# ajzhai/PEANUT

Hardware: AMD Instinct MI355X
Metric: maps/sec for 480x480x(4+N_cat) prediction fwd, batch 32 (higher is better)
Workload: dtype f32; 1 GPU; 480x480, 14-channel (4+10) partial maps -> 6-class prediction forward (PSPNet R50-V1c-D8), batch 32 per GPU, seeded random-init weights; survey_config=2, global_batch=32, parallelism=dp1 (map shards, no data-path collective)

## Files before the change

### peanut_amd/csrc/common.h

```cpp
#pragma once
#include <hip/hip_runtime.h>
#include <stdint.h>
#include <string>

#include "persistent_plan.h"

namespace peanut {

void set_error(const std::string& msg);
int fail(int code, const std::string& msg);
void note_kernel(const char* family);
const char* noted_kernel();

#define PEANUT_HIP_CHECK(expr)                                                            \
  do {                                                                                    \
    hipError_t _e = (expr);                                                               \
    if (_e != hipSuccess)                                                                 \
      return ::peanut::fail(-3, std::string(#expr) + ": " + hipGetErrorString(_e));       \
  } while (0)

struct ConvDesc {
  int cin;
  int cout;
  int kh, kw, stride, pad, dil;
// ... 94 lines not shown
  int pack_bn;
  int G;
  PersistentPlan plan;
  int code;
  const char* error;
};
struct ConvKParams;
ConvRoute conv_route(const ConvDesc& d, const ConvArgs& a, ConvKParams* params = nullptr);
ConvRoute conv_route_patch_nchw();
const char* conv_kernel_family(const ConvRoute& r);
int device_cus();
bool conv_pw_enabled();
bool conv_pw_uses_256(int cout, long long M, int mt_per_group, int bn_tile, int cin);
int conv_pw_256_min_k();
bool conv_pw_uses_256w(int cout, long long M, int mt_per_group, int bn_tile, int cin, int flush_ktiles);
bool conv_pw_narrow_tiles(int cin, int cout, long long M, int bn_tile, int mt_per_group);
bool conv_pw_uses_256p(int cout, long long M, int mt_per_group, int bn_tile, int cin, int flush_ktiles, long long in_pixels = 0);
bool gemm_skinny_takes(const ConvKParams& p, int bn_tile, size_t ws_floats);
bool conv_pw_uses_256wp(int cout, long long M, int stride, int mt_per_group, int bn_tile, int c1, int c2, int flush_ktiles);
bool conv_pw_uses_ares(int cin, int cout, long long M, int stride, bool two_source, int flush_ktiles, int bn_tile);

bool conv_patch_eligible(const ConvDesc& d, const ConvArgs& a);
bool conv_patch_nchw_eligible(const ConvDesc& d, int B, int Ho, int Wo, int creal);
int launch_conv_patch_nchw(const ConvDesc& d, const float* x_nchw, int creal, float* y, int B, int H, int W, int Ho, int Wo, hipStream_t stream);

void wino_geometry(int B, int H, int W, int dil, int* th, int* tw, long long* n_tiles, long long* m_pad, int gran = 128, int m = 4);
void wino_transform_weights(const float* w_oihw, int cout, int cin, float* out, int m = 4);
int launch_wino_input(const float* x, float* V, int B, int H, int W, int C, int dil, hipStream_t s, int gran = 128, int m = 4, long long m_pad_total = 0,
                      const DeferredSplit* df = nullptr);
bool wino_input_accepts_deferred(int B, int H, int W, int C, int dil, int gran, int m);
long long wino_deferred_count();
int launch_wino_output(const float* Mb, const float* scale, const float* shift, const float* res, float* y,
                       int B, int H, int W, int C, int dil, int relu, hipStream_t s, int gran = 128, int m = 4, long long m_pad_total = 0);

bool gemm_rs_uses_256(int cout, long long M, int mt_per_group, int bn_tile, int cin);
bool gemm_rs_uses_64(int cout, long long M, int bn_tile, int cin);
size_t sx_packed_bytes(int cin_pad, int cout, int bn_tile, int planes);
void pack_weights_sx(const float* w, int cout, int cin_real, int cin_pad, int bn_tile, int planes, float wscale, void* out);
float sx_pack_scale(const float* w, size_t n, int planes);
size_t sx_conv_packed_bytes(int cin_pad, int cout, int kh, int kw, int bn_tile, int planes);
void pack_weights_sx_conv(const float* w_oihw, int cout, int cin_real, int cin_pad, int kh, int kw, int bn_tile, int planes,
                          float wscale, void* out);

int launch_nchw_to_nhwc_pad(const float* x, float* y, int B, int C, int H, int W, int Cpad, hipStream_t s);
int launch_maxpool3x3s2(const float* x, float* y, int B, int H, int W, int C, int Ho, int Wo, hipStream_t s);
int launch_ppm_pool(const float* x, float* out, int B, int H, int W, int C, const int* scales, int nscales,
                    hipStream_t s, int scale_rows = 0);
size_t ppm_pool_scratch_floats(int B, int H, int C, const int* scales, int nscales);
int launch_ppm_pool2(const float* x, float* scratch, float* out, int B, int H, int W, int C, const int* scales,
                     int nscales, hipStream_t s, int scale_rows = 0);
int launch_ppm_upsample_concat(const float* table, float* out, int B, int H, int W, int Cp, const int* scales,
                               int nscales, int align_corners, hipStream_t s);
int launch_ppm_conv_term(const float* Q, float* R, int B, int H, int W, int C, const int* scales, int nscales,
                         int align_corners, hipStream_t s, int scale_rows = 0);
int launch_upsample_logits(const float* lo, float* out, int B, int h, int w, int K, int H, int W,
                           int align_corners, int sigmoid, hipStream_t s);

}
```

### peanut_amd/csrc/options.h

```cpp
#pragma once
#include <stdlib.h>
#include <string.h>

#include <string>

namespace peanut {

enum OptionId {
  OPT_PW_GLDS, OPT_PW256_MINK, OPT_PW256_MINTILES, OPT_PW256_PHASE, OPT_PW256_SKIP_PAD, OPT_PW256W_MINK, OPT_PW256W_MINTILES, OPT_PW256P_MINK, OPT_PW256P_MINTILES, OPT_PW256P_FLUSH, OPT_PW256P_ORDER, OPT_PW256P_STREAMK, OPT_PW256WP_MINK, OPT_PW256WP_MINTILES, OPT_PW256WP_NPRE, OPT_PW256WP_STAGGER, OPT_PW_ARES, OPT_PW_SKINNY,
  OPT_PW_ARES_MINUNITS, OPT_PATCH_MINTILES, OPT_STEM_NCHW, OPT_BN64_MAXK, OPT_PW_BN64_MAXK, OPT_PW64_MAXTILES, OPT_FP32_BK, OPT_NCHUNK, OPT_RES_PREFETCH, OPT_SPLIT_MODEL,
  OPT_RS_CONV, OPT_RS_BN64_MAXK, OPT_RS256_MINK, OPT_RS256_MINTILES, OPT_RS64_MAXK, OPT_RS64_MAXTILES,
  OPT_WINO_M, OPT_WINO_HEAD_M, OPT_WINO6_MAXDIL, OPT_WINO5_MINDIL, OPT_WINO_FLUSH_CH, OPT_WINO_MIN_CIN, OPT_WINO_NARROW_MINPIX, OPT_WINO_SMALL_MAXWG, OPT_DEFER_SPLITK,
  OPT_PPM_OVERLAP, OPT_PPM_GROUPED, OPT_PPM_TERM_ROWS, OPT_PPM_GROUP_ROWS, OPT_RCNN_WINO_M, OPT_RCNN_STEM_S2D, OPT_RCNN_RPN_FUSED, OPT_RCNN_FPN_OVERLAP, OPT_RCNN_RANK_SORT, OPT_RCNN_TOPK_SLICE, OPT_RCNN_NMS_LEVELS, OPT_FMM_LOCAL32, OPT_FMM_MAX_PASSES, OPT_FMM_BLOCKED, OPT_FMM_INNER,
  OPT_DEBUG_POISON_ALLOC,
  OPT_COUNT
};

struct OptionInfo {
  const char* key;
  long long def;
  bool upload_time;
  const char* help;
};

inline const OptionInfo* option_table() {
  static const OptionInfo t[OPT_COUNT] = {
      {"pw_glds", 1, false, "fp32 1x1 convs / grouped GEMMs on the LDS-DMA kernels of conv_pw.hip (0: conv_igemm)"},
      {"pw256_mink", 1024, false, "fewest input channels for the 256 x 128 three-stage kernel"},
      {"pw256_mintiles", 256, false, "fewest 256 x 128 tiles for that kernel"},
      {"pw256_phase", 1, false, "the two waves of a SIMD request their LDS-DMA pieces half an iteration apart"},
      {"pw256_skip_pad", 1, false, "256 x 128 kernel, grouped GEMMs: waves whose rows are all group padding issue no MFMAs (0: compute the zero rows)"},
      {"pw256w_mink", 768, false, "fewest input channels for the 256 x 256 two-stage kernel (0: off)"},
      {"pw256w_mintiles", 1536, false, "fewest 256 x 256 tiles for that kernel"},
      {"pw256p_mink", 512, false, "fewest input channels for the persistent 256 x 128 kernel (conv_pw256p.hip; 0: off)"},
      {"pw256p_mintiles", 512, false, "fewest 256 x 128 tiles for that kernel"},
      {"pw256p_flush", 512, false, "most input channels of a Winograd position GEMM (two-level accumulation) that runs on the persistent kernel (0: none)"},
      {"pw256p_order", 1, false, "persistent 256 x 128 kernel: 1 = the workgroups of an XCD walk its run of tiles side by side (neighbours share operand panels in L2), 0 = one contiguous run per workgroup"},
      {"pw256p_streamk", 1, false, "persistent 256 x 128 kernel: the tail tiles' k-tiles as one stream in equal runs per workgroup (0: every tail tile cut into the same number of parts)"},
      {"pw256wp_mink", 512, false, "fewest input channels for the persistent 256 x 256 kernel (conv_pw256wp.hip; 0: off)"},
      {"pw256wp_mintiles", 768, false, "fewest 256 x 256 tiles for that kernel"},
      {"pw256wp_npre", 0, false, "persistent 256 x 256 kernel: accumulator blocks per in-place epilogue group (2 or 4; 0 = two with a residual, four without)"},
      {"pw256wp_stagger", 0, false, "persistent 256 x 256 kernel: spread of the workgroups' start times in sleeps of ~3.4 us (their tile boundaries -- 512 KiB of epilogue traffic per CU -- then fall at different times)"},
      {"pw_ares", 1, false, "K = 128 / 256 pointwise layers on the persistent A-resident kernel (conv_pw_ares.hip)"},
      {"pw_skinny", 1, false, "grouped pointwise launches with at most 64 data rows per group (the PSP pyramid's per-scale convs and Q tables at batch 1) on the skinny weight-streaming kernel (gemm_skinny.hip: 6 KiB of LDS, fits next to any other kernel; 0: the MFMA kernels on 128-row padded tiles)"},
      {"pw_ares_minunits", 512, false, "fewest (m-tile, n-tile) units for that kernel"},
      {"patch_mintiles", 1024, false, "3x3 convs of 16 / 32 input channels on the persistent LDS-patch kernel (conv_patch.hip) from this many 8 x 16 output tiles (0: off)"},
      {"stem_nchw", 1, false, "prediction forward: the first stem conv reads the NCHW input itself (conv_patch.hip, NCHW variant) instead of a layout pass + NHWC conv (fp32 mode, when the patch kernel takes the layer)"},
      {"bn64_maxk", 256, true, "128 x 64 tiles for layers with at most this many input channels"},
      {"pw_bn64_maxk", 128, true, "pointwise layers / Winograd position GEMMs: weights PACKED 64 wide up to this many input channels (wider layers: 128-wide packing, 64-wide tiles chosen per shape)"},
      {"pw64_maxtiles", 512, false, "a 128-wide-packed pointwise layer with at most bn64_maxk input channels runs 128 x 64 tiles while its 128 x 128 tiling has fewer tiles than this (two per CU)"},
      {"fp32_bk", 0, true, "16: force 16-channel k-tiles in conv_igemm (experiment)"},
      {"nchunk", 8, false, "n-tiles per chunk of the tile order (0: n fastest over all n-tiles)"},
      {"res_prefetch", 1, false, "request the first residual rows before the last k-tile's MFMAs"},
      {"split_model", 1, false, "tail split-K plan counts CUs (1) or resident slots (0)"},
      {"rs_conv", 1, true, "emulated modes: non-pointwise convs on conv_rs.hip (0: fp32 MFMA kernel)"},
      {"rs_bn64_maxk", 128, true, "emulated modes: 128 x 64 tiles up to this many input channels"},
      {"rs256_mink", 512, false, "emulated modes: fewest input channels for the 256 x 256 kernel"},
      {"rs256_mintiles", 256, false, "emulated modes: fewest 256 x 256 tiles for it"},
      {"rs64_maxk", 512, false, "emulated modes: 64 x 64 tiles up to this many input channels"},
      {"rs64_maxtiles", 128, false, "emulated modes: ... and below this many 128-row tiles"},
      {"wino_m", 0, true, "4 / 5 / 6: force one Winograd form on every eligible layer (0: policy)"},
      {"wino_head_m", 0, true, "4 / 5 / 6: Winograd form of the PSP bottleneck (0: policy)"},
      {"wino6_maxdil", 4, true, "largest dilation that gets an F(6x6) form"},
      {"wino5_mindil", 4, true, "smallest dilation that also gets an F(5x5) form (0: none)"},
      {"wino_flush_ch", 64, true, "channels per partial sum of the position GEMMs' two-level accumulation (0: off)"},
      {"wino_min_cin", 0, true, "fewest input channels of a Winograd layer (0: the planner's policy)"},
      {"wino_narrow_minpix", 20000, false, "layers under 128 channels take their Winograd form from this many input pixels on (round 6: 100 000 -> 20 000 -- with the small-problem transforms one 720 x 720 map's layer1 conv2, 32 400 pixels, gains 5 us per layer as F(6x6); profiles/r9e)"},
      {"wino_small_maxwg", 1024, false, "Winograd transforms: launches with fewer workgroups than this of the one-thread-per-tile kernels take the small-problem variants (a workgroup per tile and 64-channel slice, a thread per line, through LDS; bit-identical; 0: never)"},
      {"defer_splitk", 1, false, "a Bottleneck conv1 whose every tile is split along k leaves its partial tiles unsummed and conv2's (small-problem) Winograd input transform sums them: one launch fewer per block at batch 1, bit-identical (0: every conv runs its own reduce); read when a (B, H, W) plan is built"},
      {"ppm_overlap", -1, false, "pyramid branch of the PSP head on a side stream: 0 / 1, -1 = by size"},
      {"ppm_grouped", -1, false, "per-scale PSP GEMMs as one grouped launch: 0 / 1, -1 = by size"},
      {"ppm_term_rows", 1, false, "folded pyramid term: one wave per output row, no barrier in the row loop (0: the workgroup-wide two-phase kernel)"},
      {"ppm_group_rows", 0, false, "pyramid pooling, row pass: rows added up per workgroup (1..5; 0 = by size: as many as still leave ~768 workgroups)"},
      {"rcnn_wino_m", 0, true, "detector front end: 4 / 5 / 6 pins one Winograd form (0: per shape)"},
      {"rcnn_stem_s2d", 1, true, "detector stem 7x7 stride 2 as a space-to-depth 4x4 conv"},
      {"rcnn_rpn_fused", 1, false, "detector: the RPN head on all five pyramid levels as one chain (five input transforms, ONE grouped Winograd GEMM, five output transforms, one objectness and one anchor-delta GEMM over all levels' rows: 12 launches instead of 25); read when a (B, H, W) plan is built"},
      {"rcnn_fpn_overlap", 0, false, "detector: the FPN output convs of p5, p4, p3 on a side stream next to the lateral / top-down chain that ends in p2's (round 5 experiment, bit-identical; measured SLOWER at batch 1, 5.70 against 5.61 ms per frame, profiles/r8: off); read when a (B, H, W) plan is built"},
      {"rcnn_rank_sort", 1, false, "detector: the RPN candidates of an image are ordered by counting the larger keys (n / 64 workgroups) instead of one workgroup's bitonic sort (round 5; same order: the keys are distinct)"},
      {"rcnn_topk_slice", 20480, false, "detector: objectness logits per workgroup of the per-level top-k (a level is cut into up to 8 ranges whose k largest are merged by counting; 0: one workgroup per level, round 4)"},
      {"rcnn_nms_levels", 1, false, "detector: the proposal NMS level by level (five 16 x 16-word suppression blocks and five scans per image side by side, post-NMS top-k by counting) instead of one score-sorted list per image (round 5; same proposals)"},
      {"fmm_local32", 1, false, "goal solver: single-precision local solve inside a tile"},
      {"fmm_max_passes", 24, false, "goal solver: hard ceiling of the second-order ordering passes; they stop as soon as a pass changes nothing (6-10 passes on the agent's 960 x 960 map; peanut_goal_converged reports whether they reached their fixed point)"},
      {"fmm_blocked", 1, false, "goal solver: a wave relaxes its 8 x 8 block of the tile to convergence between workgroup barriers (round 5; 0: one Jacobi sweep of the whole tile per barrier pair)"},
      {"fmm_inner", 48, false, "goal solver: iterations a wave spends on its block before it publishes it (blocked rounds)"},
      {"debug_poison_alloc", 0, false, "test switch: every device allocation the library makes for itself (workspace arenas, conv / Winograd / split-K scratch, the detector's and the goal solver's buffers, the map projection's arrays, uploaded weights before their copy) is filled with 0xFF bytes straight after hipMalloc -- fp32 / fp64 read NaN, int reads -1, 64-bit keys all ones -- so a kernel that reads a slot nothing wrote shows up as a changed result (tests/test_workspace_gpu.py); 0: allocations stay as the allocator returns them, no extra call"},
  };
  return t;
}

struct Options {
  long long v[OPT_COUNT];
};

inline int option_index(const char* key) {
  if (!key) return -1;
  std::string k(key);
  for (auto& c : k) c = (char)((c >= 'A' && c <= 'Z') ? c - 'A' + 'a' : c);
  if (k.rfind("peanut_", 0) == 0) k = k.substr(7);
  const OptionInfo* t = option_table();
  for (int i = 0; i < OPT_COUNT; ++i)
    if (k == t[i].key) return i;
  return -1;
}

inline Options& default_options() {
  static Options d = [] {
// ... 34 lines not shown
```

### peanut_amd/csrc/pred_api.hip

```cpp
#include <math.h>
#include <string.h>

#include <map>
#include <memory>
#include <string>
#include <vector>

#include "net_common.h"

namespace peanut {

static thread_local std::string g_err;
void set_error(const std::string& msg) { g_err = msg; }
int fail(int code, const std::string& msg) {
  g_err = msg;
  return code;
}
static thread_local const char* g_kernel = "";
void note_kernel(const char* family) { g_kernel = family; }
const char* noted_kernel() { return g_kernel; }

namespace {

enum OpKind { OP_TO_NHWC, OP_CONV, OP_CONV_NCHW, OP_MAXPOOL, OP_PPM_POOL, OP_PPM_UP, OP_PPM_TERM, OP_UPSAMPLE, OP_WINO_IN, OP_WINO_GEMM, OP_WINO_OUT };

struct Op {
  OpKind kind;
  std::string name;
  std::string kernel;
  const ConvLayer* conv = nullptr;
  Act in, in2, res, out;
  bool has_in2 = false, has_res = false;
  double flops = 0;
  double bytes = 0;
  int wino_mt_per_group = 0;
  int wino_valid_rows = 0;
  int wino_gran = 128;
  int branch = 0;
  bool fork_before = false, join_before = false;
  int group_mt = 0;
  int ppm_scale_rows = 0;
  bool defer_ok = false;
};

struct Plan {
  int B = 0, H = 0, W = 0;
  Act splitk;
  Act splitk2;
  bool keep_all = false;
  size_t bytes = 0;
  std::vector<Op> ops;
  std::map<std::string, Act> named;
};

}
}

using namespace peanut;

struct peanut_conv {
  Options opts = default_options();
  ConvLayer L;
  DevBuf ws;
  DevBuf wino_v, wino_m;
};

struct peanut_pred {
  Options opts = default_options();
  DeferredSplit deferred{};
  peanut_pred_cfg cfg{};
  int cin_pad = 0;
  std::vector<std::unique_ptr<ConvLayer>> convs;
  ConvLayer* stem[3] = {nullptr, nullptr, nullptr};
  struct Block { ConvLayer *c1, *c2, *c3, *down, *c3d; };
  std::vector<std::vector<Block>> layers;
  std::vector<ConvLayer*> ppm;
  ConvLayer* bottleneck = nullptr;
  ConvLayer* bottleneck_x = nullptr;
  std::vector<ConvLayer*> ppm_q;
  std::unique_ptr<ConvLayer> ppm_grouped, ppmq_grouped;
  ConvLayer* conv_seg = nullptr;
  int feat_channels = 0;
  bool keep_all = false;
  std::map<std::string, std::unique_ptr<Plan>> plans;
  Plan* last_plan = nullptr;
  DevBuf ws;
  bool use_graph = false;
  GraphCache graphs;
  bool probe = false;
  Plan* probe_plan = nullptr;
  std::vector<std::vector<hipEvent_t>> probe_events;
  std::vector<hipEvent_t> event_pool;
  hipStream_t side = nullptr;
  hipEvent_t ev_fork = nullptr, ev_join = nullptr;
  ~peanut_pred() {
    for (auto& v : probe_events) for (auto e : v) (void)hipEventDestroy(e);
    for (auto e : event_pool) (void)hipEventDestroy(e);
    if (ev_fork) (void)hipEventDestroy(ev_fork);
    if (ev_join) (void)hipEventDestroy(ev_join);
    if (side) (void)hipStreamDestroy(side);
  }
};

namespace {

int bn_fold(peanut_pred* h, const TensorMap& tm, const std::string& bn, int cout, float* scale, float* shift) {
  return bn_fold_eps(tm, bn, cout, h->cfg.bn_eps, scale, shift);
}

int add_conv(peanut_pred* h, const TensorMap& tm, const std::string& conv, const std::string& bn, int cin,
             int cin_pad, int cout, int k, int stride, int pad, int dil, int relu, ConvLayer** out) {
  int rc = 0;
  const int64_t wshape[4] = {cout, cin, k, k};
  const peanut_tensor* w = tm.get(conv + ".weight", 4, wshape, &rc);
// ... 271 lines not shown
      Act scr; scr.B = 1; scr.H = 1; scr.W = 1; scr.C = 0; scr.bytes = sf * sizeof(float); scr.off = ar.alloc(scr.bytes);
      op.in2 = scr; op.has_in2 = true;
      pl->ops.push_back(op);
      rel_side(scr);
    } else {
      pl->ops.push_back(op);
    }
  }
  Act table = make_act(ar, 1, 1, prow, h->cfg.head_channels);
  auto push_grouped = [&](const ConvLayer* G, const Act& in, const Act& out) {
    push_conv(*pl, G, in, nullptr, nullptr, out);
    Op& op = pl->ops.back();
    op.group_mt = srows / 128;
    op.flops = 2.0 * (double)prow * G->d.cout * G->cin_real;
  };
  if (srows) {
    push_grouped(h->ppm_grouped.get(), pooled, table);
  } else {
    size_t row0 = 0;
    for (int i = 0; i < h->cfg.n_pool_scales; ++i) {
      const int k = h->cfg.pool_scales[i];
      Act in = pooled, out = table;
      in.off = pooled.off + row0 * (size_t)x.C * sizeof(float);
      in.H = 1; in.W = k * k; in.C = x.C; in.B = B;
      out.off = table.off + row0 * (size_t)h->cfg.head_channels * sizeof(float);
      out.H = 1; out.W = k * k; out.C = h->cfg.head_channels; out.B = B;
      push_conv(*pl, h->ppm[i], in, nullptr, nullptr, out);
      row0 += (size_t)B * k * k;
    }
  }
  pl->named["ppm_table"] = table;
  rel_side(pooled);
  Act bt;
  int term_scale_rows = 0;
  if (h->bottleneck_x) {
    const int hc = h->cfg.head_channels;
    Act q = make_act(ar, 1, 1, prow, 9 * hc);
    if (srows) {
      push_grouped(h->ppmq_grouped.get(), table, q);
      term_scale_rows = srows;
    } else {
      size_t row0 = 0;
      for (int i = 0; i < h->cfg.n_pool_scales; ++i) {
        const int k = h->cfg.pool_scales[i];
        Act in = table, out = q;
        in.off = table.off + row0 * (size_t)hc * sizeof(float);
        in.H = 1; in.W = k * k; in.C = hc; in.B = B;
        out.off = q.off + row0 * (size_t)(9 * hc) * sizeof(float);
        out.H = 1; out.W = k * k; out.C = 9 * hc; out.B = B;
        push_conv(*pl, h->ppm_q[i], in, nullptr, nullptr, out);
        row0 += (size_t)B * k * k;
      }
    }
    rel_side(table);
    Act r = make_act(ar, B, x.H, x.W, hc);
    {
      Op op; op.kind = OP_PPM_TERM; op.name = "ppm_conv_term"; op.kernel = "ppm_conv_term"; op.in = q; op.out = r; op.ppm_scale_rows = term_scale_rows;
      op.bytes = (double)q.bytes + (double)r.bytes;
      pl->ops.push_back(op);
    }
    rel_side(q);
    const size_t side_end = pl->ops.size();
    bt = make_act(ar, B, x.H, x.W, h->bottleneck_x->d.cout);
    push_conv(*pl, h->bottleneck_x, x, nullptr, &r, bt, &ar);
    if (overlap) {
      for (size_t i = side_first; i < side_end; ++i) pl->ops[i].branch = 1;
      pl->ops[side_first].fork_before = true;
      for (size_t i = side_end; i < pl->ops.size(); ++i)
        if (pl->ops[i].has_res) { pl->ops[i].join_before = true; break; }
      for (const auto& t : side_bufs) rel(t);
    }
    rel(r);
  } else {
    Act up = make_act(ar, B, x.H, x.W, h->cfg.n_pool_scales * h->cfg.head_channels);
    { Op op; op.kind = OP_PPM_UP; op.name = "ppm_upsample_concat"; op.kernel = "ppm_upsample_concat"; op.in = table; op.out = up; pl->ops.push_back(op); }
    rel(table);
    bt = make_act(ar, B, x.H, x.W, h->bottleneck->d.cout);
    push_conv(*pl, h->bottleneck, x, &up, nullptr, bt);
    rel(up);
  }
  pl->named["bottleneck"] = bt;
  rel(x);
  Act lo = make_act(ar, B, bt.H, bt.W, h->conv_seg->d.cout);
  push_conv(*pl, h->conv_seg, bt, nullptr, nullptr, lo);
  pl->named["logits_lowres"] = lo;
  rel(bt);
  {
    Op op; op.kind = OP_UPSAMPLE; op.name = "upsample_logits"; op.kernel = "upsample_logits"; op.in = lo;
    op.bytes = (double)lo.bytes + (double)B * H * W * h->conv_seg->d.cout * 4.0;
    pl->ops.push_back(op);
  }
  rel(lo);
  for (Op& op : pl->ops) {
    if (op.kind != OP_CONV && op.kind != OP_WINO_GEMM) continue;
    int scale_rows[8];
    op.kernel = conv_kernel_family(conv_route(conv_op_desc(op), conv_op_args(h, *pl, op, kPlanningBase, scale_rows)));
  }
  return pl;
}

}

static size_t plan_high_water(const Plan& pl) {
  size_t hw = 0;
  auto upd = [&](const Act& a) { if (a.bytes && a.off + Arena::round_up(a.bytes) > hw) hw = a.off + Arena::round_up(a.bytes); };
  for (const auto& op : pl.ops) {
    upd(op.in); upd(op.in2); upd(op.res); upd(op.out);
  }
  for (const auto& kv : pl.named) upd(kv.second);
  upd(pl.splitk);
  upd(pl.splitk2);
  return hw;
}

static Plan* get_plan(peanut_pred* h, int B, int H, int W) {
  if (B <= 0 || H < 16 || W < 16) { set_error("forward: need B >= 1 and H, W >= 16"); return nullptr; }
  const std::string key = std::to_string(B) + "x" + std::to_string(H) + "x" + std::to_string(W) + (h->keep_all ? "k" : "");
  auto it = h->plans.find(key);
  if (it == h->plans.end()) {
    auto pl = build_plan(h, B, H, W);
    pl->bytes = plan_high_water(*pl);
    it = h->plans.emplace(key, std::move(pl)).first;
  }
  return it->second.get();
}

static int run_op(peanut_pred* h, const Plan& pl, const Op& op, const float* in_dev, float* out_dev, int sigmoid,
                  hipStream_t s) {
  char* base = (char*)h->ws.p;
  auto P = [&](const Act& a) { return (float*)(base + a.off); };
  switch (op.kind) {
    case OP_TO_NHWC:
      return launch_nchw_to_nhwc_pad(in_dev, P(op.out), pl.B, h->cfg.in_channels, pl.H, pl.W, h->cin_pad, s);
    case OP_CONV_NCHW:
      return launch_conv_patch_nchw(op.conv->d, in_dev, h->cfg.in_channels, P(op.out), pl.B, pl.H, pl.W, op.out.H, op.out.W, s);
    case OP_CONV: {
      int scale_rows[8];
      ConvArgs a = conv_op_args(h, pl, op, base, scale_rows);
      if (op.defer_ok) a.defer = &h->deferred;
      return launch_conv(op.conv->d, a, s);
    }
    case OP_WINO_IN: {
      const int rc = launch_wino_input(P(op.in), P(op.out), op.in.B, op.in.H, op.in.W, op.in.C, op.conv->d.dil, s, op.wino_gran, op.conv->wino_m, 0,
                                       h->deferred.valid ? &h->deferred : nullptr);
      h->deferred.valid = false;
      return rc;
    }
    case OP_WINO_GEMM: {
      int scale_rows[8];
      return launch_conv(op.conv->wino, conv_op_args(h, pl, op, base, scale_rows), s);
    }
    case OP_WINO_OUT:
      return launch_wino_output(P(op.in), op.conv->d.scale, op.conv->d.shift, op.has_res ? P(op.res) : nullptr, P(op.out),
                                op.out.B, op.out.H, op.out.W, op.out.C, op.conv->d.dil, op.conv->d.relu, s, op.wino_gran, op.conv->wino_m);
    case OP_MAXPOOL:
      return launch_maxpool3x3s2(P(op.in), P(op.out), op.in.B, op.in.H, op.in.W, op.in.C, op.out.H, op.out.W, s);
    case OP_PPM_POOL:
      return launch_ppm_pool2(P(op.in), op.has_in2 ? P(op.in2) : nullptr, P(op.out), op.in.B, op.in.H, op.in.W, op.in.C,
                              h->cfg.pool_scales, h->cfg.n_pool_scales, s, op.ppm_scale_rows);
    case OP_PPM_UP:
      return launch_ppm_upsample_concat(P(op.in), P(op.out), op.out.B, op.out.H, op.out.W, h->cfg.head_channels,
                                        h->cfg.pool_scales, h->cfg.n_pool_scales, h->cfg.align_corners, s);
    case OP_PPM_TERM:
      return launch_ppm_conv_term(P(op.in), P(op.out), op.out.B, op.out.H, op.out.W, h->cfg.head_channels,
                                  h->cfg.pool_scales, h->cfg.n_pool_scales, h->cfg.align_corners, s, op.ppm_scale_rows);
    case OP_UPSAMPLE:
      return launch_upsample_logits(P(op.in), out_dev, op.in.B, op.in.H, op.in.W, op.in.C, pl.H, pl.W,
                                    h->cfg.align_corners, sigmoid, s);
  }
  return fail(PEANUT_EINVAL, "unknown op");
}

extern "C" {

const char* peanut_last_error(void) { return g_err.c_str(); }
const char* peanut_last_conv_kernel(void) { return noted_kernel(); }
int peanut_abi_version(void) { return 19; }
const char* peanut_build_arch(void) { return "gfx950"; }
#ifndef PEANUT_SOURCE_HASH
#define PEANUT_SOURCE_HASH ""
#endif
const char* peanut_source_hash(void) { return PEANUT_SOURCE_HASH; }

namespace {
int option_lookup(const char* key, const char* who) {
// ... 118 lines not shown
    const int64_t wshape[4] = {hc, cat, 3, 3};
    const peanut_tensor* w = tm.get("decode_head.bottleneck.conv.weight", 4, wshape, &rc);
    if (!w) return rc;
    std::vector<float> scale(hc), shift(hc);
    if ((rc = bn_fold(h.get(), tm, "decode_head.bottleneck.bn", hc, scale.data(), shift.data()))) return rc;
    std::vector<float> wx((size_t)hc * inplanes * 9);
    for (int n = 0; n < hc; ++n)
      memcpy(&wx[(size_t)n * inplanes * 9], &w->data[(size_t)n * cat * 9], (size_t)inplanes * 9 * sizeof(float));
    {
      auto L = std::make_unique<ConvLayer>();
      L->name = "decode_head.bottleneck.conv[x]";
      if ((rc = upload_conv(*L, wx.data(), scale.data(), shift.data(), hc, inplanes, inplanes, 3, 3, 1, 1, 1, 1, cfg->precision))) return rc;
      if (cfg->conv_algo == PEANUT_ALGO_AUTO && wino_eligible(inplanes, hc, 3, 3, 1, 1, 1, cfg->precision) &&
          (rc = upload_wino_forms(*L, wx.data(), scale.data(), shift.data(), hc, inplanes, inplanes, 1, 1, 1, cfg->precision,
                                  wino_head_tile(cfg->precision))))
        return rc;
      h->bottleneck_x = L.get();
      h->convs.push_back(std::move(L));
    }
    std::vector<float> wq((size_t)9 * hc * hc);
    for (int s = 0; s < cfg->n_pool_scales; ++s) {
      for (int tap = 0; tap < 9; ++tap)
        for (int n = 0; n < hc; ++n)
          for (int c = 0; c < hc; ++c)
            wq[((size_t)tap * hc + n) * hc + c] = scale[n] * w->data[((size_t)n * cat + inplanes + (size_t)s * hc + c) * 9 + tap];
      auto L = std::make_unique<ConvLayer>();
      L->name = "decode_head.bottleneck.conv[ppm" + std::to_string(s) + "]";
      if ((rc = upload_conv(*L, wq.data(), nullptr, nullptr, 9 * hc, hc, hc, 1, 1, 1, 0, 1, 0, PEANUT_PREC_FP32))) return rc;
      h->ppm_q.push_back(L.get());
      h->convs.push_back(std::move(L));
    }
  }
  if ((rc = add_conv(h.get(), tm, "decode_head.conv_seg", "", hc, hc, cfg->num_classes, 1, 1, 0, 1, 0, &h->conv_seg))) return rc;
  if (cfg->fold_ppm) {
    h->ppm_grouped = build_grouped(h->ppm, "decode_head.psp_modules.*.1.conv", &rc);
    if (rc) return rc;
    h->ppmq_grouped = build_grouped(h->ppm_q, "decode_head.bottleneck.conv[ppm*]", &rc);
    if (rc) return rc;
  }
  PEANUT_HIP_CHECK(hipDeviceSynchronize());
  *out = h.release();
  return 0;
}

void peanut_pred_destroy(peanut_pred_t* h) { delete h; }

size_t peanut_pred_workspace_bytes(peanut_pred_t* h, int B, int H, int W) {
  if (!h) return 0;
  OptionScope option_scope(&h->opts);
  Plan* pl = get_plan(h, B, H, W);
  return pl ? pl->bytes : 0;
}

double peanut_pred_flops_per_map(peanut_pred_t* h, int H, int W) {
  if (!h) return 0;
  OptionScope option_scope(&h->opts);
  Plan* pl = get_plan(h, 1, H, W);
  if (!pl) return 0;
  double f = 0;
  for (const auto& op : pl->ops) f += op.flops;
  return f;
}

int peanut_pred_debug_keep(peanut_pred_t* h, int keep) {
  if (!h) return fail(PEANUT_EINVAL, "null handle");
  h->keep_all = keep != 0;
// ... 200 lines not shown
```

### peanut_amd/csrc/winograd.hip

```cpp
#include <stdlib.h>

#include <atomic>

#include "common.h"
#include "conv_common.h"

namespace peanut {

namespace {

template <typename V>
__device__ __forceinline__ V fmak(V a, float k, V c) { return __builtin_elementwise_fma(a, (V)k, c); }

__device__ __forceinline__ void bt6(const f32x4 d0, const f32x4 d1, const f32x4 d2, const f32x4 d3, const f32x4 d4,
                                    const f32x4 d5, f32x4& t0, f32x4& t1, f32x4& t2, f32x4& t3, f32x4& t4, f32x4& t5) {
#pragma clang fp contract(off)
  const f32x4 a = fmak(d2, -2.25f, d4), b = fmak(d3, 0.75f, -1.6875f * d1);
  const f32x4 c = fmak(d2, -0.5625f, d4), e = fmak(d3, 1.5f, -0.84375f * d1);
  t0 = fmak(d0, 1.265625f, fmak(d2, -2.8125f, d4));
  t1 = a + b;
  t2 = a - b;
  t3 = c + e;
  t4 = c - e;
  t5 = fmak(d1, 1.265625f, fmak(d3, -2.8125f, d5));
// ... 245 lines not shown
    auto res_column = [&](int j, f32x2 (&dst)[6]) __attribute__((always_inline)) {
      const int c = c0 + j * g.d;
#pragma unroll
      for (int a = 0; a < 6; ++a) {
        const int r = r0 + a * g.d;
        const bool ok = c < g.W && r < g.H;
        const size_t off = ok ? (img + (size_t)r * g.W + c) * g.C + ng * 2 : 0;
        dst[a] = *reinterpret_cast<const f32x2*>(res + off);
      }
    };
    if constexpr (RES) res_column(0, rn);
#pragma unroll
    for (int j = 0; j < 6; ++j) {
      f32x2 rc[6];
      if constexpr (RES) {
#pragma unroll
        for (int a = 0; a < 6; ++a) rc[a] = rn[a];
        if (j + 1 < 6) res_column(j + 1, rn);
      }
      f32x2 o[6];
      at8(q[0][j], q[1][j], q[2][j], q[3][j], q[4][j], q[5][j], q[6][j], q[7][j], o[0], o[1], o[2], o[3], o[4], o[5]);
      const int c = c0 + j * g.d;
      if (c >= g.W) continue;
#pragma unroll
      for (int a = 0; a < 6; ++a) {
        const int r = r0 + a * g.d;
        if (r >= g.H) continue;
        const size_t off = (img + (size_t)r * g.W + c) * g.C + ng * 2;
        f32x2 v = o[a] * sc + sh;
        if constexpr (RES) v += rc[a];
        if (relu) { v.x = relu_keep_nan(v.x); v.y = relu_keep_nan(v.y); }
        *reinterpret_cast<f32x2*>(y + off) = v;
      }
    }
  }
}

__device__ __forceinline__ void bt7(const f32x2 d0, const f32x2 d1, const f32x2 d2, const f32x2 d3, const f32x2 d4, const f32x2 d5,
                                    const f32x2 d6, f32x2& t0, f32x2& t1, f32x2& t2, f32x2& t3, f32x2& t4, f32x2& t5, f32x2& t6) {
  const f32x2 r0 = d5 - 0.75f * d0 + 0.25f * d1 + 3.75f * d2 - 1.25f * d3 - 3.f * d4;
  const f32x2 r1 = d5 + 1.5f * d1 + 2.5f * (d2 - d3 - d4);
  const f32x2 r2 = d5 - 1.5f * d1 + 3.5f * (d2 - d4) + 0.5f * d3;
  const f32x2 r3 = d5 + 0.75f * d1 + 0.5f * d2 - 3.25f * d3 - 2.f * d4;
  const f32x2 r4 = d5 - 0.75f * d1 + d2 + 2.75f * d3 - 4.f * d4;
  const f32x2 r5 = d5 + 0.25f * d1 - 1.25f * d3;
  const f32x2 r6 = d6 - 0.75f * d1 + 0.25f * d2 + 3.75f * d3 - 1.25f * d4 - 3.f * d5;
  t0 = r0; t1 = r1; t2 = r2; t3 = r3; t4 = r4; t5 = r5; t6 = r6;
}

__device__ __forceinline__ void at7(const f32x2 m0, const f32x2 m1, const f32x2 m2, const f32x2 m3, const f32x2 m4, const f32x2 m5,
                                    const f32x2 m6, f32x2& y0, f32x2& y1, f32x2& y2, f32x2& y3, f32x2& y4) {
  const f32x2 s1 = m1 + m2, d1 = m1 - m2, s2 = m3 + m4, d2 = m3 - m4;
  y0 = m0 + s1 + s2 + m5;
  y1 = 0.5f * d1 + d2 + 3.f * m5;
  y2 = 0.25f * s1 + s2 + 9.f * m5;
  y3 = 0.125f * d1 + d2 + 27.f * m5;
  y4 = 0.0625f * s1 + s2 + 81.f * m5 + m6;
}

__global__ __launch_bounds__(256) void wino5_input_kernel(const float* __restrict__ x, float* __restrict__ V, const WinoGeom g) {
  const int groups = g.C >> 1;
  const long long total = g.n_tiles * groups;
  for (long long idx = (long long)blockIdx.x * blockDim.x + threadIdx.x; idx < total;
       idx += (long long)gridDim.x * blockDim.x) {
    int cg;
    long long tile;
// ... 451 lines not shown
  } else if (m == 6) hipLaunchKernelGGL(wino6_input_kernel, dim3(grid_for(total)), dim3(256), 0, s, x, V, g);
  else if (m == 5) hipLaunchKernelGGL(wino5_input_kernel, dim3(grid_for(total)), dim3(256), 0, s, x, V, g);
  else hipLaunchKernelGGL(wino_input_kernel, dim3(grid_for(total)), dim3(256), 0, s, x, V, g);
  hipError_t e = hipGetLastError();
  if (e != hipSuccess) return fail(-3, std::string("wino_input launch: ") + hipGetErrorString(e));
  return 0;
}

int launch_wino_output(const float* Mb, const float* scale, const float* shift, const float* res, float* y,
                       int B, int H, int W, int C, int dil, int relu, hipStream_t s, int gran, int m, long long m_pad_total) {
  if (C % 4 || m < 4 || m > 6) return fail(-2, "wino_output: channels must be a multiple of 4, tiles 4x4, 5x5 or 6x6");
  WinoGeom g{B, H, W, C, dil, 0, 0, 0, 0};
  wino_geometry(B, H, W, dil, &g.th, &g.tw, &g.n_tiles, &g.m_pad, gran, m);
  if (m_pad_total > 0) g.m_pad = m_pad_total;
  const long long total = g.n_tiles * (m == 4 ? C / 4 : C / 2);
  if (const int lanes = wino_small_lanes(g.n_tiles, C, m)) {
    const unsigned grid = (unsigned)(g.n_tiles * (C / (lanes * (m == 4 ? 4 : 2))));
#define PEANUT_WINO_SMALL_OUT(K, R, L, T) hipLaunchKernelGGL((K<R, L>), dim3(grid), dim3(T), 0, s, Mb, scale, shift, res, y, g, relu)
    if (m == 6 && lanes == 32) { if (res) PEANUT_WINO_SMALL_OUT(wino6_output_small_kernel, true, 32, 256); else PEANUT_WINO_SMALL_OUT(wino6_output_small_kernel, false, 32, 256); }
    else if (m == 6) { if (res) PEANUT_WINO_SMALL_OUT(wino6_output_small_kernel, true, 16, 128); else PEANUT_WINO_SMALL_OUT(wino6_output_small_kernel, false, 16, 128); }
    else if (lanes == 32) { if (res) PEANUT_WINO_SMALL_OUT(wino4_output_small_kernel, true, 32, 192); else PEANUT_WINO_SMALL_OUT(wino4_output_small_kernel, false, 32, 192); }
    else { if (res) PEANUT_WINO_SMALL_OUT(wino4_output_small_kernel, true, 16, 96); else PEANUT_WINO_SMALL_OUT(wino4_output_small_kernel, false, 16, 96); }
#undef PEANUT_WINO_SMALL_OUT
  } else if (m == 6 && res) hipLaunchKernelGGL(wino6_output_kernel<true>, dim3(grid_for(total)), dim3(256), 0, s, Mb, scale, shift, res, y, g, relu);
  else if (m == 6) hipLaunchKernelGGL(wino6_output_kernel<false>, dim3(grid_for(total)), dim3(256), 0, s, Mb, scale, shift, res, y, g, relu);
  else if (m == 5) hipLaunchKernelGGL(wino5_output_kernel, dim3(grid_for(total)), dim3(256), 0, s, Mb, scale, shift, res, y, g, relu);
  else if (res) hipLaunchKernelGGL(wino_output_kernel<true>, dim3(grid_for(total)), dim3(256), 0, s, Mb, scale, shift, res, y, g, relu);
  else hipLaunchKernelGGL(wino_output_kernel<false>, dim3(grid_for(total)), dim3(256), 0, s, Mb, scale, shift, res, y, g, relu);
  hipError_t e = hipGetLastError();
  if (e != hipSuccess) return fail(-3, std::string("wino_output launch: ") + hipGetErrorString(e));
  return 0;
}

}
```

Before: 888.8 maps/s.

## Fuse conv_seg 1x1 classifier into F(6x6) Winograd output transform of PSP bottleneck

```diff
diff --git a/peanut_amd/csrc/common.h b/peanut_amd/csrc/common.h
--- a/peanut_amd/csrc/common.h
+++ b/peanut_amd/csrc/common.h
@@ -150,6 +150,9 @@
 long long wino_deferred_count();
 int launch_wino_output(const float* Mb, const float* scale, const float* shift, const float* res, float* y,
                        int B, int H, int W, int C, int dil, int relu, hipStream_t s, int gran = 128, int m = 4, long long m_pad_total = 0);
+bool wino_output_seg_takes(int B, int H, int W, int C, int dil, int m, int ncls);
+int launch_wino6_output_seg(const float* Mb, const float* scale, const float* shift, const float* res, const float* wseg, const float* bseg,
+                            float* lo, int B, int H, int W, int C, int dil, int ncls, int relu, hipStream_t s, int gran = 128);
 
 bool gemm_rs_uses_256(int cout, long long M, int mt_per_group, int bn_tile, int cin);
 bool gemm_rs_uses_64(int cout, long long M, int bn_tile, int cin);
diff --git a/peanut_amd/csrc/options.h b/peanut_amd/csrc/options.h
--- a/peanut_amd/csrc/options.h
+++ b/peanut_amd/csrc/options.h
@@ -11,7 +11,7 @@
   OPT_PW_ARES_MINUNITS, OPT_PATCH_MINTILES, OPT_STEM_NCHW, OPT_BN64_MAXK, OPT_PW_BN64_MAXK, OPT_PW64_MAXTILES, OPT_FP32_BK, OPT_NCHUNK, OPT_RES_PREFETCH, OPT_SPLIT_MODEL,
   OPT_RS_CONV, OPT_RS_BN64_MAXK, OPT_RS256_MINK, OPT_RS256_MINTILES, OPT_RS64_MAXK, OPT_RS64_MAXTILES,
   OPT_WINO_M, OPT_WINO_HEAD_M, OPT_WINO6_MAXDIL, OPT_WINO5_MINDIL, OPT_WINO_FLUSH_CH, OPT_WINO_MIN_CIN, OPT_WINO_NARROW_MINPIX, OPT_WINO_SMALL_MAXWG, OPT_DEFER_SPLITK,
-  OPT_PPM_OVERLAP, OPT_PPM_GROUPED, OPT_PPM_TERM_ROWS, OPT_PPM_GROUP_ROWS, OPT_RCNN_WINO_M, OPT_RCNN_STEM_S2D, OPT_RCNN_RPN_FUSED, OPT_RCNN_FPN_OVERLAP, OPT_RCNN_RANK_SORT, OPT_RCNN_TOPK_SLICE, OPT_RCNN_NMS_LEVELS, OPT_FMM_LOCAL32, OPT_FMM_MAX_PASSES, OPT_FMM_BLOCKED, OPT_FMM_INNER,
+  OPT_PPM_OVERLAP, OPT_PPM_GROUPED, OPT_PPM_TERM_ROWS, OPT_PPM_GROUP_ROWS, OPT_SEG_FUSED, OPT_RCNN_WINO_M, OPT_RCNN_STEM_S2D, OPT_RCNN_RPN_FUSED, OPT_RCNN_FPN_OVERLAP, OPT_RCNN_RANK_SORT, OPT_RCNN_TOPK_SLICE, OPT_RCNN_NMS_LEVELS, OPT_FMM_LOCAL32, OPT_FMM_MAX_PASSES, OPT_FMM_BLOCKED, OPT_FMM_INNER,
   OPT_DEBUG_POISON_ALLOC,
   OPT_COUNT
 };
@@ -72,6 +72,7 @@
       {"ppm_grouped", -1, false, "per-scale PSP GEMMs as one grouped launch: 0 / 1, -1 = by size"},
       {"ppm_term_rows", 1, false, "folded pyramid term: one wave per output row, no barrier in the row loop (0: the workgroup-wide two-phase kernel)"},
       {"ppm_group_rows", 0, false, "pyramid pooling, row pass: rows added up per workgroup (1..5; 0 = by size: as many as still leave ~768 workgroups)"},
+      {"seg_fused", 1, false, "prediction forward: conv_seg inside the F(6x6) output transform of the PSP bottleneck (winograd.hip: wino6_output_seg_kernel) -- the bottleneck's output is neither written nor read back; not in debug (keep_all) plans (0: the output transform stores it and conv_seg runs as its own GEMM; 2: as 1, and a debug plan runs the fused transform too, next to the separate ops, into the named tensor logits_lowres_fused -- test hook); read when a (B, H, W) plan is built"},
       {"rcnn_wino_m", 0, true, "detector front end: 4 / 5 / 6 pins one Winograd form (0: per shape)"},
       {"rcnn_stem_s2d", 1, true, "detector stem 7x7 stride 2 as a space-to-depth 4x4 conv"},
       {"rcnn_rpn_fused", 1, false, "detector: the RPN head on all five pyramid levels as one chain (five input transforms, ONE grouped Winograd GEMM, five output transforms, one objectness and one anchor-delta GEMM over all levels' rows: 12 launches instead of 25); read when a (B, H, W) plan is built"},
diff --git a/peanut_amd/csrc/pred_api.hip b/peanut_amd/csrc/pred_api.hip
--- a/peanut_amd/csrc/pred_api.hip
+++ b/peanut_amd/csrc/pred_api.hip
@@ -40,6 +40,7 @@
   bool fork_before = false, join_before = false;
   int group_mt = 0;
   int ppm_scale_rows = 0;
+  bool seg_fused = false;
   bool defer_ok = false;
 };
 
@@ -80,6 +81,7 @@
   std::vector<ConvLayer*> ppm_q;
   std::unique_ptr<ConvLayer> ppm_grouped, ppmq_grouped;
   ConvLayer* conv_seg = nullptr;
+  DevBuf seg_wb;
   int feat_channels = 0;
   bool keep_all = false;
   std::map<std::string, std::unique_ptr<Plan>> plans;
@@ -417,6 +419,7 @@
   pl->named["ppm_table"] = table;
   rel_side(pooled);
   Act bt;
+  bool seg_ok = false, seg_fused = false;
   int term_scale_rows = 0;
   if (h->bottleneck_x) {
     const int hc = h->cfg.head_channels;
@@ -446,8 +449,36 @@
     }
     rel_side(q);
     const size_t side_end = pl->ops.size();
-    bt = make_act(ar, B, x.H, x.W, h->bottleneck_x->d.cout);
+    {
+      const ConvLayer* L = h->bottleneck_x;
+      const ConvDesc& sd = h->conv_seg->d;
+      const bool wino = L->has_wino && (long long)B * x.H * x.W >= wino_min_pixels(L->d.cin);
+      seg_ok = wino && wino_pick_form(L, B, x.H, x.W)->wino_m == 6 && sd.kh == 1 && sd.kw == 1 && sd.stride == 1 && sd.pad == 0 && !sd.relu &&
+               sd.cin == L->d.cout && wino_output_seg_takes(B, x.H, x.W, L->d.cout, L->d.dil, 6, sd.cout);
+      seg_fused = seg_ok && opt(OPT_SEG_FUSED) != 0 && !h->keep_all;
+    }
+    bt = make_act(ar, B, x.H, x.W, seg_fused ? h->conv_seg->d.cout : h->bottleneck_x->d.cout);
     push_conv(*pl, h->bottleneck_x, x, nullptr, &r, bt, &ar);
+    auto make_seg_fused = [&](Op& o, const Act& logits) {
+      const ConvLayer* L = o.conv;
+      int th, tw;
+      long long n_tiles, m_pad;
+      wino_geometry(B, x.H, x.W, L->d.dil, &th, &tw, &n_tiles, &m_pad, o.wino_gran, 6);
+      o.seg_fused = true;
+      o.out = logits;
+      o.name = L->name + "[wino6_out+conv_seg]";
+      o.kernel = "wino6_output_seg";
+      o.flops = 2.0 * (double)B * x.H * x.W * L->d.cout * h->conv_seg->d.cout;
+      o.bytes = 64.0 * (double)n_tiles * L->d.cout * 4 + (double)r.bytes + (double)logits.bytes + (double)h->seg_wb.bytes;
+    };
+    if (seg_fused) make_seg_fused(pl->ops.back(), bt);
+    if (seg_ok && h->keep_all && opt(OPT_SEG_FUSED) == 2) {
+      Op twin = pl->ops.back();
+      Act lo2 = make_act(ar, B, x.H, x.W, h->conv_seg->d.cout);
+      make_seg_fused(twin, lo2);
+      pl->ops.push_back(twin);
+      pl->named["logits_lowres_fused"] = lo2;
+    }
     if (overlap) {
       for (size_t i = side_first; i < side_end; ++i) pl->ops[i].branch = 1;
       pl->ops[side_first].fork_before = true;
@@ -464,12 +495,18 @@
     push_conv(*pl, h->bottleneck, x, &up, nullptr, bt);
     rel(up);
   }
-  pl->named["bottleneck"] = bt;
-  rel(x);
-  Act lo = make_act(ar, B, bt.H, bt.W, h->conv_seg->d.cout);
-  push_conv(*pl, h->conv_seg, bt, nullptr, nullptr, lo);
+  Act lo;
+  if (seg_fused) {
+    rel(x);
+    lo = bt;
+  } else {
+    pl->named["bottleneck"] = bt;
+    rel(x);
+    lo = make_act(ar, B, bt.H, bt.W, h->conv_seg->d.cout);
+    push_conv(*pl, h->conv_seg, bt, nullptr, nullptr, lo);
+    rel(bt);
+  }
   pl->named["logits_lowres"] = lo;
-  rel(bt);
   {
     Op op; op.kind = OP_UPSAMPLE; op.name = "upsample_logits"; op.kernel = "upsample_logits"; op.in = lo;
     op.bytes = (double)lo.bytes + (double)B * H * W * h->conv_seg->d.cout * 4.0;
@@ -536,6 +573,12 @@
       return launch_conv(op.conv->wino, conv_op_args(h, pl, op, base, scale_rows), s);
     }
     case OP_WINO_OUT:
+      if (op.seg_fused) {
+        const int ncls = h->conv_seg->d.cout, npad = (ncls + 7) / 8 * 8;
+        const float* wseg = (const float*)h->seg_wb.p;
+        return launch_wino6_output_seg(P(op.in), op.conv->d.scale, op.conv->d.shift, P(op.res), wseg, wseg + (size_t)npad * op.conv->d.cout, P(op.out),
+                                       op.out.B, op.out.H, op.out.W, op.conv->d.cout, op.conv->d.dil, ncls, op.conv->d.relu, s, op.wino_gran);
+      }
       return launch_wino_output(P(op.in), op.conv->d.scale, op.conv->d.shift, op.has_res ? P(op.res) : nullptr, P(op.out),
                                 op.out.B, op.out.H, op.out.W, op.out.C, op.conv->d.dil, op.conv->d.relu, s, op.wino_gran, op.conv->wino_m);
     case OP_MAXPOOL:
@@ -720,6 +763,19 @@
     }
   }
   if ((rc = add_conv(h.get(), tm, "decode_head.conv_seg", "", hc, hc, cfg->num_classes, 1, 1, 0, 1, 0, &h->conv_seg))) return rc;
+  {
+    const int64_t wshape[4] = {cfg->num_classes, hc, 1, 1}, bshape[1] = {cfg->num_classes};
+    const peanut_tensor* w = tm.get("decode_head.conv_seg.weight", 4, wshape, &rc);
+    if (!w) return rc;
+    const peanut_tensor* b = tm.get("decode_head.conv_seg.bias", 1, bshape, &rc);
+    if (!b) return rc;
+    const int npad = (cfg->num_classes + 7) / 8 * 8;
+    std::vector<float> wb((size_t)npad * hc + npad, 0.f);
+    memcpy(wb.data(), w->data, (size_t)cfg->num_classes * hc * sizeof(float));
+    memcpy(wb.data() + (size_t)npad * hc, b->data, (size_t)cfg->num_classes * sizeof(float));
+    if ((rc = h->seg_wb.ensure(wb.size() * sizeof(float)))) return rc;
+    PEANUT_HIP_CHECK(hipMemcpy(h->seg_wb.p, wb.data(), wb.size() * sizeof(float), hipMemcpyHostToDevice));
+  }
   if (cfg->fold_ppm) {
     h->ppm_grouped = build_grouped(h->ppm, "decode_head.psp_modules.*.1.conv", &rc);
     if (rc) return rc;
diff --git a/peanut_amd/csrc/winograd.hip b/peanut_amd/csrc/winograd.hip
--- a/peanut_amd/csrc/winograd.hip
+++ b/peanut_amd/csrc/winograd.hip
@@ -301,6 +301,104 @@
         if (relu) { v.x = relu_keep_nan(v.x); v.y = relu_keep_nan(v.y); }
         *reinterpret_cast<f32x2*>(y + off) = v;
       }
+    }
+  }
+}
+
+template <int NC>
+__global__ __launch_bounds__(256) void wino6_output_seg_kernel(const float* __restrict__ Mb, const float* __restrict__ scale,
+                                                               const float* __restrict__ shift, const float* __restrict__ res,
+                                                               const float* __restrict__ wseg, const float* __restrict__ bseg,
+                                                               float* __restrict__ lo, const WinoGeom g, int relu, int ncls) {
+  extern __shared__ float seg_lds[];
+  const int ldc = g.C + 4;
+  float* park = seg_lds;
+  float* part = seg_lds + 36 * ldc;
+  const int ng = threadIdx.x;
+  const long long tile = blockIdx.x;
+  int b, oy, ox, ty, tx;
+  decode_tile(g, tile, b, oy, ox, ty, tx);
+  const int r0 = oy + g.d * 6 * ty, c0 = ox + g.d * 6 * tx;
+  if (r0 >= g.H || c0 >= g.W) return;
+  const size_t img = (size_t)b * g.H * g.W;
+  {
+    const float* mb = Mb + (size_t)tile * g.C + ng * 2;
+    const size_t pos_stride = (size_t)g.m_pad * g.C;
+    f32x2 q[8][6];
+#pragma unroll
+    for (int i = 0; i < 8; ++i) {
+      const float* s = mb + (size_t)(i * 8) * pos_stride;
+      f32x2 m[8];
+#pragma unroll
+      for (int j = 0; j < 8; ++j) m[j] = __builtin_nontemporal_load(reinterpret_cast<const f32x2*>(s + j * pos_stride));
+      at8(m[0], m[1], m[2], m[3], m[4], m[5], m[6], m[7], q[i][0], q[i][1], q[i][2], q[i][3], q[i][4], q[i][5]);
+    }
+    const f32x2 sc = *reinterpret_cast<const f32x2*>(scale + ng * 2);
+    const f32x2 sh = *reinterpret_cast<const f32x2*>(shift + ng * 2);
+    f32x2 rn[6];
+    auto res_column = [&](int j, f32x2 (&dst)[6]) __attribute__((always_inline)) {
+      const int c = c0 + j * g.d;
+#pragma unroll
+      for (int a = 0; a < 6; ++a) {
+        const int r = r0 + a * g.d;
+        const bool ok = c < g.W && r < g.H;
+        const size_t off = ok ? (img + (size_t)r * g.W + c) * g.C + ng * 2 : 0;
+        dst[a] = *reinterpret_cast<const f32x2*>(res + off);
+      }
+    };
+    res_column(0, rn);
+#pragma unroll
+    for (int j = 0; j < 6; ++j) {
+      f32x2 rc[6];
+#pragma unroll
+      for (int a = 0; a < 6; ++a) rc[a] = rn[a];
+      if (j + 1 < 6) res_column(j + 1, rn);
+      f32x2 o[6];
+      at8(q[0][j], q[1][j], q[2][j], q[3][j], q[4][j], q[5][j], q[6][j], q[7][j], o[0], o[1], o[2], o[3], o[4], o[5]);
+#pragma unroll
+      for (int a = 0; a < 6; ++a) {
+        f32x2 v = o[a] * sc + sh;
+        v += rc[a];
+        if (relu) { v.x = relu_keep_nan(v.x); v.y = relu_keep_nan(v.y); }
+        *reinterpret_cast<f32x2*>(park + (a * 6 + j) * ldc + ng * 2) = v;
+      }
+    }
+  }
+  __syncthreads();
+  const int wave = __builtin_amdgcn_readfirstlane((int)(threadIdx.x >> 6)), lane = threadIdx.x & 63;
+  const int waves = blockDim.x >> 6;
+  const float* row = park + (lane < 36 ? lane : 35) * ldc + wave * 128;
+  const int n_out = 36 * ncls;
+  for (int k0 = 0; k0 < ncls; k0 += NC) {
+    const float* wk = wseg + (size_t)k0 * g.C + wave * 128;
+    f32x2 acc[NC];
+#pragma unroll
+    for (int k = 0; k < NC; ++k) acc[k] = f32x2{0.f, 0.f};
+#pragma unroll 4
+    for (int c = 0; c < 128; c += 4) {
+      const f32x4 xv = *reinterpret_cast<const f32x4*>(row + c);
+      const f32x2 x01 = {xv.x, xv.y}, x23 = {xv.z, xv.w};
+#pragma unroll
+      for (int k = 0; k < NC; ++k) {
+        const float* w = wk + (size_t)k * g.C + c;
+        acc[k] = __builtin_elementwise_fma(x01, *reinterpret_cast<const f32x2*>(w), acc[k]);
+        acc[k] = __builtin_elementwise_fma(x23, *reinterpret_cast<const f32x2*>(w + 2), acc[k]);
+      }
+    }
+    if (k0) __syncthreads();
+    if (lane < 36) {
+#pragma unroll
+      for (int k = 0; k < NC; ++k) part[(wave * 36 + lane) * NC + k] = acc[k].x + acc[k].y;
+    }
+    __syncthreads();
+    for (int u = threadIdx.x; u < n_out; u += blockDim.x) {
+      const int p = u / ncls, k = u - p * ncls;
+      if (k < k0 || k >= k0 + NC) continue;
+      const int r = r0 + (p / 6) * g.d, c = c0 + (p % 6) * g.d;
+      if (r >= g.H || c >= g.W) continue;
+      float v = part[p * NC + (k - k0)];
+      for (int w = 1; w < waves; ++w) v += part[(w * 36 + p) * NC + (k - k0)];
+      lo[(img + (size_t)r * g.W + c) * ncls + k] = v + bseg[k];
     }
   }
 }
@@ -818,4 +916,41 @@
   return 0;
 }
 
-}
+bool wino_output_seg_takes(int B, int H, int W, int C, int dil, int m, int ncls) {
+  if (m != 6 || C % 128 || C < 128 || C > 512 || ncls < 1 || ncls > 32) return false;
+  int th, tw;
+  long long n_tiles, m_pad;
+  wino_geometry(B, H, W, dil, &th, &tw, &n_tiles, &m_pad, 128, 6);
+  return n_tiles <= 0x7fffffffLL;
+}
+
+namespace {
+template <int NC>
+int launch_seg(const float* Mb, const float* scale, const float* shift, const float* res, const float* wseg, const float* bseg, float* lo,
+               const WinoGeom& g, int relu, int ncls, hipStream_t s) {
+  const size_t lds = ((size_t)36 * (g.C + 4) + (size_t)(g.C / 128) * 36 * NC) * sizeof(float);
+  static bool raised = false;
+  if (!raised) {
+    hipError_t e = hipFuncSetAttribute(reinterpret_cast<const void*>(wino6_output_seg_kernel<NC>), hipFuncAttributeMaxDynamicSharedMemorySize, 80 * 1024);
+    if (e != hipSuccess) return fail(-3, std::string("hipFuncSetAttribute: ") + hipGetErrorString(e));
+    raised = true;
+  }
+  hipLaunchKernelGGL(wino6_output_seg_kernel<NC>, dim3((unsigned)g.n_tiles), dim3(g.C / 2), lds, s, Mb, scale, shift, res, wseg, bseg, lo, g, relu, ncls);
+  hipError_t e = hipGetLastError();
+  if (e != hipSuccess) return fail(-3, std::string("wino_output_seg launch: ") + hipGetErrorString(e));
+  return 0;
+}
+}
+
+int launch_wino6_output_seg(const float* Mb, const float* scale, const float* shift, const float* res, const float* wseg, const float* bseg,
+                            float* lo, int B, int H, int W, int C, int dil, int ncls, int relu, hipStream_t s, int gran) {
+  if (!res || !wino_output_seg_takes(B, H, W, C, dil, 6, ncls)) return fail(-2, "wino_output_seg: needs a residual, 128..512 channels in whole waves, 1..32 classes");
+  WinoGeom g{B, H, W, C, dil, 0, 0, 0, 0};
+  wino_geometry(B, H, W, dil, &g.th, &g.tw, &g.n_tiles, &g.m_pad, gran, 6);
+  if (ncls <= 2) return launch_seg<2>(Mb, scale, shift, res, wseg, bseg, lo, g, relu, ncls, s);
+  if (ncls <= 4) return launch_seg<4>(Mb, scale, shift, res, wseg, bseg, lo, g, relu, ncls, s);
+  if (ncls <= 6) return launch_seg<6>(Mb, scale, shift, res, wseg, bseg, lo, g, relu, ncls, s);
+  return launch_seg<8>(Mb, scale, shift, res, wseg, bseg, lo, g, relu, ncls, s);
+}
+
+}
```

Measured after the change: 892.6 maps/s (median of 6 runs). About the same (+0.4%).
